# PKU-Alignment/Safe-Policy-Optimization

Hardware: NVIDIA H100
Metric: env-steps/sec PPO-Lag SafetyPointGoal1 @1024 envs/GPU (higher is better)
Workload: dtype f32

## Files before the change

safe-policy-optimization_b200/csrc/spo_update.cu:

```cuda
#include "spo_update_kernel.cuh"

#ifdef SPO_PHASE_TIMERS
extern "C" int spo_debug_phase_cycles(unsigned long long* out_16x24, int reset) {
  SPO_CUDA_TRY(cudaMemcpyFromSymbol(out_16x24, g_phase_cycles, sizeof(unsigned long long) * 16 * 24));
  if (reset) {
    unsigned long long z[16 * 24] = {0};
    SPO_CUDA_TRY(cudaMemcpyToSymbol(g_phase_cycles, z, sizeof(z)));
  }
  return SPO_OK;
}
#endif

extern "C" int spo_comm_slot_floats(const spo_dims* d, int* slot_floats) {
  int rc = spo_check_dims(d);
  if (rc) return rc;
  SPO_REQUIRE(slot_floats, SPO_ERR_INVALID_ARG, "spo_comm_slot_floats: null output");
  const int nt1 = d->obs_dim <= 64 ? 1 : 2;
  *slot_floats = NQ * dp_slot_words(nt1) * 2;
  return SPO_OK;
}

extern "C" int spo_pg_update(const spo_dims* d, float* params, float* adam_m, float* adam_v, int* adam_t,
                             const spo_batch* data, const int64_t* perm, int64_t perm_len, int batch,
                             spo_loss_kind kind, const spo_hparams* hp, spo_update_ctrl* ctrl, void* stream) {
// ... 31 lines not shown
    a.kind = SPO_LOSS_PPO_CLIP;
    a.hp.clip_lo = -INFINITY;
    a.hp.clip_hi = INFINITY;
  }
  if (comm && comm->world > 1) {
    SPO_REQUIRE(comm->rank >= 0 && comm->rank < comm->world && comm->world <= 16 && comm->grad_bufs,
                SPO_ERR_INVALID_ARG, "spo_pg_update_dp: bad spo_comm (world=%d rank=%d)", comm->world, comm->rank);
    SPO_REQUIRE(d->act_dim <= 8, SPO_ERR_UNSUPPORTED,
                "spo_pg_update_dp: act_dim=%d > 8 is single-GPU only (the cross-GPU update supports act_dim <= 8)", d->act_dim);
    a.comm = *comm;
  } else {
    a.comm.world = 1;
  }
  cudaStream_t st = static_cast<cudaStream_t>(stream);
  const bool dp = a.comm.world > 1;
  if (d->act_dim > 8) return spo_update_launch_wide(d->obs_dim <= 64 ? 1 : 2, &a, st);
  if (d->obs_dim <= 64) return dp ? launch_update<1, 8, true>(a, st) : launch_update<1, 8, false>(a, st);
  return dp ? launch_update<2, 8, true>(a, st) : launch_update<2, 8, false>(a, st);
}
```

safe-policy-optimization_b200/csrc/spo_update_kernel.cuh:

```cuda
#pragma once
#include <cooperative_groups.h>
#include <stdlib.h>
#include "spo_common.cuh"
#include "spo_mma.cuh"

namespace cg = cooperative_groups;

#ifdef SPO_PHASE_TIMERS
__device__ unsigned long long g_phase_cycles[16][24];
#define PHASE_MARK(idx)                                                   \
  do {                                                                    \
    if (tid == 0) {                                                       \
      const long long now__ = clock64();                                  \
      sm_phase__[idx] += static_cast<unsigned long long>(now__ - phase_t__); \
      phase_t__ = now__;                                                  \
    }                                                                     \
  } while (0)
#else
#define PHASE_MARK(idx) do { } while (0)
#endif

namespace {

constexpr int UT = 256;
constexpr int NQ = 4;
constexpr int SL = SPO_HID / NQ;
constexpr int NCTA = 3 * NQ;
constexpr int LDA = 72;
constexpr int LDS = 40;
constexpr float kLogSqrt2Pi = 0.91893853320467274178f;

template <int AC>
struct UpdShape {
  static_assert(AC == 8 || AC == 16, "action capacity 8 or 16");
  static constexpr int AUXW = 3 * AC + 4;
  static constexpr int AUX_LOGP = AC, AUX_ADV = AC + 1, AUX_TGT = AC + 2, AUX_OMEAN = AC + 4, AUX_OSTD = 2 * AC + 4;
  static constexpr int AUX_IT = (AUXW + 3) / 4;
  static constexpr int SP_B1 = 0, SP_B2 = SL, SP_W3 = 2 * SL, SP_B3 = 2 * SL + AC * SL, SP_LS = SP_B3 + AC;
  static constexpr int SPN = SP_LS + AC;
  static constexpr int SPT = (SPN + UT - 1) / UT;
  static constexpr int YQ = SPO_ROWS * AC;
  static constexpr int DH = AC / 4;
};
static_assert(UpdShape<8>::SPN == 176 && UpdShape<8>::SPT == 1 && UpdShape<16>::SPN == 320 && UpdShape<16>::SPT == 2, "layout");

__host__ __device__ constexpr int upd_ldx(int nt1) { return 64 * nt1 + 8; }
__host__ __device__ constexpr int dp_slot_words(int nt1) { return UT * 4 * (1 + nt1) + UT; }

template <int N> struct IC { static constexpr int value = N; };

struct UpdArgs {
  float *params, *adam_m, *adam_v;
  int* adam_t;
  spo_batch data;
  const int64_t* perm;
  int64_t perm_len;
  int batch, kind, D, A;
  int actor_only;
  spo_hparams hp;
  spo_update_ctrl* ctrl;
  spo_comm comm;
};

__device__ __forceinline__ uint32_t smem_u32(const void* p) { return static_cast<uint32_t>(__cvta_generic_to_shared(p)); }
__device__ __forceinline__ uint32_t mapa(uint32_t addr, uint32_t rank) {
  uint32_t r;
  asm volatile("mapa.shared::cluster.u32 %0, %1, %2;" : "=r"(r) : "r"(addr), "r"(rank));
  return r;
// ... 18 lines not shown
  while (!ok) {
    asm volatile("{ .reg .pred p; mbarrier.try_wait.parity.acquire.cluster.shared::cta.b64 p, [%1], %2; selp.u32 %0, 1, 0, p; }"
                 : "=r"(ok) : "r"(a), "r"(parity) : "memory");
  }
}
__device__ __forceinline__ void st_async16(uint32_t remote_dst, float4 v, uint32_t remote_bar) {
  asm volatile("st.async.shared::cluster.mbarrier::complete_tx::bytes.v4.b32 [%0], {%1, %2, %3, %4}, [%5];"
               ::"r"(remote_dst), "r"(__float_as_uint(v.x)), "r"(__float_as_uint(v.y)), "r"(__float_as_uint(v.z)),
               "r"(__float_as_uint(v.w)), "r"(remote_bar) : "memory");
}
__device__ __forceinline__ void bulk_push(uint32_t remote_dst, const void* local_src, uint32_t bytes, uint32_t remote_bar) {
  asm volatile("cp.async.bulk.shared::cluster.shared::cta.mbarrier::complete_tx::bytes [%0], [%1], %2, [%3];"
               ::"r"(remote_dst), "r"(smem_u32(local_src)), "r"(bytes), "r"(remote_bar) : "memory");
}
__device__ __forceinline__ void fence_proxy_async() { asm volatile("fence.proxy.async.shared::cta;" ::: "memory"); }
__device__ __forceinline__ void cp_async8(void* smem, const void* gmem) {
  asm volatile("cp.async.ca.shared.global [%0], [%1], 8;\n" ::"r"(smem_u32(smem)), "l"(gmem));
}
__device__ __forceinline__ void cp_async_commit() { asm volatile("cp.async.commit_group;\n" ::); }
__device__ __forceinline__ void cp_async_wait_all() { asm volatile("cp.async.wait_group 0;\n" ::: "memory"); }
__device__ __forceinline__ void st_ll(float2* p, float v, unsigned seq) {
  asm volatile("st.relaxed.sys.global.v2.b32 [%0], {%1, %2};" ::"l"(p), "r"(__float_as_uint(v)), "r"(seq) : "memory");
}

struct AdamK {
  float w1, b2, w2, ibc2s, eps, ss;
};
__device__ __forceinline__ float sqrt_approx(float x) {
  float r;
  asm("sqrt.approx.f32 %0, %1;" : "=f"(r) : "f"(x));
  return r;
}
__device__ __forceinline__ float adam_update(float p, float g, float& m, float& v, const AdamK& k) {
  m = fmaf(k.w1, __fsub_rn(g, m), m);
  v = __fadd_rn(__fmul_rn(v, k.b2), __fmul_rn(__fmul_rn(k.w2, g), g));
// ... 135 lines not shown
#pragma unroll
  for (int ks = 0; ks < 8; ++ks) {
    uint32_t ah[4], al[4], bh[2], bl[2];
#pragma unroll
    for (int i = 0; i < 4; ++i) spo_split_tf32(af[ks][i], ah[i], al[i]);
    spo_split_tf32(bf[ks][0], bh[0], bl[0]);
    spo_split_tf32(bf[ks][1], bh[1], bl[1]);
    spo_mma_tf32(c_lh, al, bh);
    spo_mma_tf32(c_hl, ah, bl);
    spo_mma_tf32(c_hh, ah, bh);
  }
#pragma unroll
  for (int e = 0; e < 4; ++e) acc[0][e] += (c_lh[e] + c_hl[e]) + c_hh[e];
}

template <int NT1, int AC, bool DP>
__global__ void __launch_bounds__(UT, 1) spo_update_kernel(const UpdArgs a) {
  static_assert(!(DP && AC != 8), "the cross-GPU gradient slots hold one small parameter per thread");
  using S = UpdShape<AC>;
  constexpr int AUXW = S::AUXW, AUX_LOGP = S::AUX_LOGP, AUX_ADV = S::AUX_ADV, AUX_TGT = S::AUX_TGT, AUX_OMEAN = S::AUX_OMEAN,
                AUX_OSTD = S::AUX_OSTD;
  constexpr int SP_B1 = S::SP_B1, SP_B2 = S::SP_B2, SP_W3 = S::SP_W3, SP_B3 = S::SP_B3, SP_LS = S::SP_LS, SPN = S::SPN;
  constexpr int SPT = S::SPT, YQ = S::YQ, DH = S::DH;
  extern __shared__ __align__(16) float smem[];
  __shared__ __align__(8) uint64_t bar_h1, bar_dh, bar_y, bar_ss[2];
  __shared__ int comm_dead;
  cg::cluster_group cluster = cg::this_cluster();
  const unsigned rank = cluster.block_rank();
  const int tid = threadIdx.x, lane = tid & 31, wid = tid >> 5;
  spo_update_ctrl* ctrl = a.ctrl;
  if (*reinterpret_cast<volatile int*>(&ctrl->stop)) return;

  const int D = a.D, A = a.A;
  constexpr int ldx = upd_ldx(NT1);
  const bool idle = rank >= NCTA;
  const int net = idle ? 2 : static_cast<int>(rank) / NQ;
  const int q = static_cast<int>(rank) % NQ;
  const unsigned grp0 = static_cast<unsigned>(net * NQ);
  const bool is_actor = (net == 0);
  const bool active = !idle && !(is_actor && a.kind == SPO_LOSS_CRITIC_ONLY) && !(!is_actor && a.actor_only);
  const SpoNetOff off = spo_net_off(D, A, net);
  const int O = off.out;
  const int g8 = lane >> 2, t4 = lane & 3;

  float* p = smem;
  int64_t* idxbuf = reinterpret_cast<int64_t*>(p); p += 2 * 2 * SPO_ROWS;
  float* lsc = p; p += 4 * AC;
  float* adk = p; p += 16;
  float* w1s = p; p += SL * ldx;
  float* w2s = p; p += SL * LDA;
  float* sp = p;  p += SPN;
  float* gsmall = p; p += SPN;
  float* x = p;   p += SPO_ROWS * ldx;
  float* aux = p; p += SPO_ROWS * AUXW;
  float* h1 = p;  p += NQ * H1Q;
  float* h2s = p; p += SPO_ROWS * LDS;
  float* dz2s = p; p += SPO_ROWS * LDS;
  float* dz1s = p; p += SPO_ROWS * LDS;
  float* yblk = p; p += NQ * YQ;
  float* y = p;   p += SPO_ROWS * AC;
  float* dy = p;  p += SPO_ROWS * AC;
  float* dls = p; p += SPO_ROWS * AC;
  float* dh1b = p; p += NQ * H1Q;
  float* dh1in = p; p += NQ * H1Q;
  float* red = p; p += 64;
  float* bk = p;  p += 3 * (4 * NT1 + 1) * UT;
  float* xin = p; p += 2 * 16 * 4;
  float* b1s = sp + SP_B1; float* b2s = sp + SP_B2; float* w3s = sp + SP_W3; float* b3 = sp + SP_B3; float* log_std = sp + SP_LS;

  const int tps = (a.batch + SPO_ROWS - 1) / SPO_ROWS;
  const int64_t n_steps = (a.perm_len + a.batch - 1) / a.batch;
  const int64_t n_tiles = n_steps * tps;

  if (tid == 0) {
    comm_dead = 0;
    mbar_init(&bar_h1, 1);
    mbar_init(&bar_dh, 1);
    mbar_init(&bar_y, 1);
    mbar_init(&bar_ss[0], 1);
    mbar_init(&bar_ss[1], 1);
    asm volatile("fence.mbarrier_init.release.cluster;" ::: "memory");
    if (!idle) { mbar_expect_tx(&bar_ss[0], (NCTA - 1) * 16); mbar_expect_tx(&bar_ss[1], (NCTA - 1) * 16); }
    for (int b = 0; b < 2; ++b) {
      adk[8 * b + 0] = static_cast<float>(1.0 - static_cast<double>(a.hp.beta1));
      adk[8 * b + 1] = a.hp.beta2;
      adk[8 * b + 2] = static_cast<float>(1.0 - static_cast<double>(a.hp.beta2));
      adk[8 * b + 4] = a.hp.adam_eps;
    }
    if (active) {
      mbar_expect_tx(&bar_h1, (NQ - 1) * H1Q * 4);
      mbar_expect_tx(&bar_dh, (NQ - 1) * H1Q * 4);
      mbar_expect_tx(&bar_y, (NQ - 1) * YQ * 4);
    }
  }

  bool sp_valid = false, sp_counted = false;
  int sp_goff = 0;
  if (tid < SPN && !idle) {
    const int i = tid;
    sp_counted = true;
    if (i < SP_B2) { sp_valid = true; sp_goff = off.b1 + SL * q + i; }
    else if (i < SP_W3) { sp_valid = true; sp_goff = off.b2 + SL * q + (i - SP_B2); }
    else if (i < SP_B3) { const int o = (i - SP_W3) / SL, kk = (i - SP_W3) % SL; sp_valid = o < O; sp_goff = off.w3 + o * SPO_HID + SL * q + kk; }
    else if (i < SP_LS) { const int o = i - SP_B3; sp_valid = o < O; sp_goff = off.b3 + o; sp_counted = (q == 0); }
    else { const int j = i - SP_LS; sp_valid = is_actor && j < A; sp_goff = off.log_std + j; sp_counted = (q == 0); }
  }
  float sp_m = 0.f, sp_v = 0.f;
// ... 20 lines not shown
      const int j = i / LDA, k = i - j * LDA;
      w2s[i] = (k < SPO_HID) ? __ldg(a.params + off.w2 + (SL * q + j) * SPO_HID + k) : 0.f;
    }
    if (tid < SPN) {
      sp[tid] = sp_valid ? a.params[sp_goff] : 0.f;
      gsmall[tid] = 0.f;
      if (sp_valid) { sp_m = a.adam_m[sp_goff]; sp_v = a.adam_v[sp_goff]; }
    }
    if constexpr (SPT > 1) {
      if (tid + UT < SPN) {
        sp[tid + UT] = sp_valid1 ? a.params[sp_goff1] : 0.f;
        gsmall[tid + UT] = 0.f;
        if (sp_valid1) { sp_m1 = a.adam_m[sp_goff1]; sp_v1 = a.adam_v[sp_goff1]; }
      }
    }
    for (int i = tid; i < SPO_ROWS * ldx; i += UT) x[i] = 0.f;
    for (int i = tid; i < SPO_ROWS * AUXW; i += UT) aux[i] = 0.f;
  }
  float mW2[4], vW2[4], mW1[NT1][4], vW1[NT1][4];
  auto frag_jk = [&](int e, int ntile, int& j, int& k) { j = g8 + ((e >> 1) << 3); k = 8 * ntile + 2 * t4 + (e & 1); };
#pragma unroll
  for (int e = 0; e < 4; ++e) {
    int j, k;
    frag_jk(e, wid, j, k);
    mW2[e] = active ? a.adam_m[off.w2 + (SL * q + j) * SPO_HID + k] : 0.f;
    vW2[e] = active ? a.adam_v[off.w2 + (SL * q + j) * SPO_HID + k] : 0.f;
#pragma unroll
    for (int i = 0; i < NT1; ++i) {
      frag_jk(e, wid + 8 * i, j, k);
      const bool ok = active && k < D;
      mW1[i][e] = ok ? a.adam_m[off.w1 + (SL * q + j) * D + k] : 0.f;
      vW1[i][e] = ok ? a.adam_v[off.w1 + (SL * q + j) * D + k] : 0.f;
    }
  }
  const int t0 = a.adam_t[net];
  double b1pow = pow(static_cast<double>(a.hp.beta1), static_cast<double>(t0));
  double b2pow = pow(static_cast<double>(a.hp.beta2), static_cast<double>(t0));
  const float lr = (net == 0) ? a.hp.lr_actor : (net == 1 ? a.hp.lr_reward : a.hp.lr_cost);
  const float extra_sumsq = (is_actor && q == 0 && a.kind == SPO_LOSS_CRITIC_ONLY && !idle) ? ctrl->extra_sumsq : 0.f;
  const float vcoef = (net == 1) ? a.hp.value_coef : 1.f;
  const float reg = is_actor ? 0.f : __fmul_rn(vcoef, __fmul_rn(a.hp.critic_l2, 2.f));

  constexpr int PF_MAX = 4 * NT1;
  const bool vec_rows = (D & 3) == 0;
  float xr[4 * PF_MAX];
#pragma unroll
  for (int i = 0; i < 4 * PF_MAX; ++i) xr[i] = 0.f;
  constexpr int AUX_IT = S::AUX_IT;
  float auxr[AUX_IT];
#pragma unroll
  for (int i = 0; i < AUX_IT; ++i) auxr[i] = 0.f;
  const int r4s = tid >> 2, q4s = tid & 3;
  const int aux_per = !is_actor ? 1 : A + 2 + (a.kind == SPO_LOSS_FOCOPS ? 2 * A : 0);
  auto aux_slot = [&](int c) {
    if (!is_actor) return AUX_TGT;
    if (c < A) return c;
    if (c == A) return AUX_LOGP;
    if (c == A + 1) return AUX_ADV;
    if (c < 2 * A + 2) return AUX_OMEAN + (c - A - 2);
    return AUX_OSTD + (c - 2 * A - 2);
  };
  auto aux_by_row = [&](int c) { return is_actor && (c < A || c >= A + 2); };
  auto aux_src = [&](int c) -> const float* {
    if (!is_actor) return (net == 1) ? a.data.target_r : a.data.target_c;
    if (c < A) return a.data.act + c;
    if (c == A) return a.data.logp;
    if (c == A + 1) return a.data.adv;
    if (c < 2 * A + 2) return a.data.old_mean + (c - A - 2);
    return a.data.old_std + (c - 2 * A - 2);
  };
  const float* aux_src0 = aux_src(q4s < aux_per ? q4s : 0);
  const int aux_mul0 = aux_by_row(q4s) ? A : 1;
  const int aux_slot0 = aux_slot(q4s < aux_per ? q4s : 0);

  int64_t step_idx = 0;
#ifdef SPO_PHASE_TIMERS
  __shared__ unsigned long long sm_phase__[24];
  if (tid < 24) sm_phase__[tid] = 0ull;
  long long phase_t__ = clock64();
#endif
  auto tile_after = [&](int64_t step, int sub, int n, int64_t& step_o, int& sub_o) {
    step_o = step; sub_o = sub;
    for (int i = 0; i < n; ++i)
      if (++sub_o == tps) { sub_o = 0; ++step_o; }
  };
  auto load_next = [&](int64_t qt, int64_t step, int sub) {
    if (!active || qt >= n_tiles) return;
    int64_t rs = a.perm_len - step * a.batch;
    if (rs > a.batch) rs = a.batch;
    int rows = static_cast<int>(rs) - sub * SPO_ROWS;
    rows = rows < 0 ? 0 : (rows > SPO_ROWS ? SPO_ROWS : rows);
    const uint32_t* ridx = reinterpret_cast<const uint32_t*>(idxbuf + (qt & 1) * SPO_ROWS);
    const uint32_t Du = static_cast<uint32_t>(D);
    const bool rv = r4s < rows;
    const uint32_t g = rv ? ridx[2 * r4s] : 0u;
    const float* rowp = a.data.obs + static_cast<size_t>(g) * Du;
    if (vec_rows) {
#pragma unroll
      for (int it = 0; it < PF_MAX; ++it) {
        const int c = q4s + 4 * it;
        float4 v = make_float4(0.f, 0.f, 0.f, 0.f);
        if (rv && 4 * c < D) v = __ldg(reinterpret_cast<const float4*>(rowp) + c);
        xr[4 * it] = v.x; xr[4 * it + 1] = v.y; xr[4 * it + 2] = v.z; xr[4 * it + 3] = v.w;
      }
    } else {
#pragma unroll
      for (int it = 0; it < 4 * PF_MAX; ++it) {
        const int c = q4s + 4 * it;
        xr[it] = (rv && c < D) ? __ldg(rowp + c) : 0.f;
      }
    }
    auxr[0] = (rv && q4s < aux_per) ? __ldg(aux_src0 + static_cast<size_t>(g) * static_cast<uint32_t>(aux_mul0)) : 0.f;
    if (aux_per > 4) {
#pragma unroll
      for (int i = 1; i < AUX_IT; ++i) {
        const int c = q4s + 4 * i;
        float v = 0.f;
        if (rv && c < aux_per) v = __ldg(aux_src(c) + static_cast<size_t>(g) * static_cast<uint32_t>(aux_by_row(c) ? A : 1));
        auxr[i] = v;
      }
    }
  };
  auto store_next = [&]() {
    if (!active) return;
    if (vec_rows) {
#pragma unroll
      for (int it = 0; it < PF_MAX; ++it) {
        const int c = q4s + 4 * it;
        if (4 * c < D) *reinterpret_cast<float4*>(x + r4s * ldx + 4 * c) = make_float4(xr[4 * it], xr[4 * it + 1], xr[4 * it + 2], xr[4 * it + 3]);
      }
    } else {
#pragma unroll
      for (int it = 0; it < 4 * PF_MAX; ++it) {
        const int c = q4s + 4 * it;
        if (c < D) x[r4s * ldx + c] = xr[it];
      }
    }
    if (q4s < aux_per) aux[r4s * AUXW + aux_slot0] = auxr[0];
    if (aux_per > 4) {
#pragma unroll
      for (int i = 1; i < AUX_IT; ++i) {
        const int c = q4s + 4 * i;
        if (c < aux_per) aux[r4s * AUXW + aux_slot(c)] = auxr[i];
      }
    }
  };
  auto fetch_idx = [&](int64_t qt, int64_t step, int sub) {
    if (!active || qt >= n_tiles) return;
    const int64_t first = step * a.batch + sub * SPO_ROWS;
    int64_t rs = a.perm_len - first;
    if (rs > a.batch - sub * SPO_ROWS) rs = a.batch - sub * SPO_ROWS;
    if (tid < SPO_ROWS && tid < rs) cp_async8(idxbuf + (qt & 1) * SPO_ROWS + tid, a.perm + first + tid);
  };
  auto colsum_into = [&](const float* buf, float* dst) {
    const int c = tid >> 4, rg = tid & 15;
    float s = 0.f;
#pragma unroll
    for (int i = 0; i < 4; ++i) s += buf[(rg + 16 * i) * LDS + c];
    s += __shfl_xor_sync(0xffffffffu, s, 1);
    s += __shfl_xor_sync(0xffffffffu, s, 2);
    s += __shfl_xor_sync(0xffffffffu, s, 4);
    s += __shfl_xor_sync(0xffffffffu, s, 8);
    if (rg == 0) dst[c] += s;
  };

  {
    int64_t st; int sb;
    fetch_idx(0, 0, 0);
    cp_async_commit();
    cp_async_wait_all();
    __syncthreads();
    load_next(0, 0, 0);
    tile_after(0, 0, 1, st, sb);
    fetch_idx(1, st, sb);
    cp_async_commit();
  }

  uint32_t ph_x = 0;
  uint32_t tcount = 0;

  float gW2[1][4], gW1[NT1][4];
#pragma unroll
  for (int e = 0; e < 4; ++e) {
    gW2[0][e] = 0.f;
#pragma unroll
    for (int i = 0; i < NT1; ++i) gW1[i][e] = 0.f;
  }
  double acc_loss = 0.0;
  float step_loss = 0.f, step_aux0 = 0.f, step_aux1 = 0.f;

  const int world = DP ? a.comm.world : 1, me = DP ? a.comm.rank : 0;
// ... 186 lines not shown
      frag_jk(e, wid, j, kc);
      *reinterpret_cast<float2*>(w2s + j * LDA + kc) = w2v[e >> 1];
    }
    if (own0) { sp[tid] = spv; gsmall[tid] = 0.f; }
    if constexpr (SPT > 1) {
      if (tid + UT < SPN) { sp[tid + UT] = spv1; gsmall[tid + UT] = 0.f; }
    }
#pragma unroll
    for (int e = 0; e < 4; ++e) gW2[0][e] = 0.f;
  };

  int64_t step = 0;
  int sub = 0;
  auto next_tile = [&]() { if (++sub == tps) { sub = 0; ++step; } };
  for (int64_t qt = 0; qt < n_tiles; ++qt, next_tile()) {
    int64_t rs64 = a.perm_len - step * a.batch;
    if (rs64 > a.batch) rs64 = a.batch;
    const int rows_step = static_cast<int>(rs64);
    int rows = rows_step - sub * SPO_ROWS;
    rows = rows < 0 ? 0 : (rows > SPO_ROWS ? SPO_ROWS : rows);
    const bool last_tile = (sub == tps - 1);
    const float inv_b = __fdiv_rn(1.f, static_cast<float>(rows_step));
    const unsigned seq = static_cast<unsigned>(a.comm.seq_base + static_cast<unsigned long long>(step_idx) + 1ull);
    const int par = static_cast<int>(step_idx & 1);
    auto stage_next = [&]() {
      int64_t st; int sb;
      tile_after(step, sub, 1, st, sb);
      load_next(qt + 1, st, sb);
      PHASE_MARK(18);
      tile_after(st, sb, 1, st, sb);
      fetch_idx(qt + 2, st, sb);
      cp_async_commit();
    };
    auto dp_push = [&](const float* vals, auto n_c, int w0) {
      constexpr int n = decltype(n_c)::value;
      const size_t base = ((static_cast<size_t>(seq & 1u) * world + me) * NCTA + rank) * DPW;
      for (int r = 0; r < world; ++r) {
        if (r == me) continue;
        float2* dst = reinterpret_cast<float2*>(a.comm.grad_bufs[r]) + base;
#pragma unroll
        for (int i = 0; i < n; ++i) st_ll(dst + (w0 + i) * UT + tid, vals[i], seq);
      }
    };
    auto dp_sum_wide = [&](float (&g2)[4], float (&g1)[NT1][4], float& gs) {
      constexpr int NW = 4 * (1 + NT1) + 1, G = 3;
      const unsigned limit = a.comm.spin_limit ? a.comm.spin_limit : 400000000u;
      const float inv_w = __fdiv_rn(1.f, static_cast<float>(world));
      float val[NW];
// ... 91 lines not shown
          }
        }
#pragma unroll
        for (int i = 0; i < NW; ++i) acc[i] += v[i];
      }
      const float inv_w = __fdiv_rn(1.f, static_cast<float>(world));
#pragma unroll
      for (int e = 0; e < 4; ++e) {
        g2[e] = __fmul_rn(acc[e], inv_w);
#pragma unroll
        for (int i = 0; i < NT1; ++i) g1[i][e] = __fmul_rn(acc[4 * (1 + i) + e], inv_w);
      }
      gs = __fmul_rn(acc[NW - 1], inv_w);
    };

    store_next();
    __syncthreads();
    PHASE_MARK(0);

    if (active) layer1();
    PHASE_MARK(2);
    const bool defer = pending;
    float clip = 1.f;
    if (pending) {
      pending = false;
      step_barrier_wait();
      PHASE_MARK(9);
      clip = resolve_clip(pend_par);
      if (active) {
        if (clip < 1.f) {
          __syncthreads();
// ... 57 lines not shown
#pragma unroll
      for (int h = 0; h < DH; ++h) piv[h] = 1.f;
#pragma unroll
      for (int h = 0; h < DH; ++h) pls[h] = 0.f;
      {
        const float* axp = aux + r4 * AUXW;
        if (is_actor) {
#pragma unroll
          for (int h = 0; h < DH; ++h) {
            const int j = k4 + 4 * h;
            if (j < A) { pa[h] = axp[j]; psd[h] = lsc[4 * j]; piv[h] = lsc[4 * j + 1]; pls[h] = lsc[4 * j + 2]; }
          }
          plogp = axp[AUX_LOGP];
          padv = axp[AUX_ADV];
        } else if (k4 == 0) {
          ptgt = axp[AUX_TGT];
        }
      }
      if (defer) log_loss(pend_par, pend_inv_b);
      if (last_tile) {
        float* kp = adk + 8 * par;
        if (tid == UT - 32) {
          b1pow *= static_cast<double>(a.hp.beta1);
          kp[5] = -__fdiv_rn(lr, static_cast<float>(1.0 - b1pow));
        } else if (tid == UT - 64) {
          b2pow *= static_cast<double>(a.hp.beta2);
          kp[3] = __fdiv_rn(1.f, sqrtf(static_cast<float>(1.0 - b2pow)));
        }
      }
      mbar_wait(&bar_y, ph_x);
      if (tid == 0) mbar_expect_tx(&bar_y, (NQ - 1) * YQ * 4);
// ... 261 lines not shown
          v[d] = *reinterpret_cast<const float4*>(src + r4 * SL + 4 * k4);
        }
        float4 s4 = v[0];
#pragma unroll
        for (int d = 1; d < NQ; ++d) { s4.x += v[d].x; s4.y += v[d].y; s4.z += v[d].z; s4.w += v[d].w; }
        const float4 h = *reinterpret_cast<const float4*>(h1 + q * H1Q + r4 * SL + ((4 * k4) ^ (((r4 >> 1) & 1) << 3)));
        s4.x *= (1.f - h.x * h.x); s4.y *= (1.f - h.y * h.y); s4.z *= (1.f - h.z * h.z); s4.w *= (1.f - h.w * h.w);
        *reinterpret_cast<float4*>(dz1s + r4 * LDS + 4 * k4) = s4;
      }
      __syncthreads();
      PHASE_MARK(11);
#pragma unroll
      for (int i = 0; i < NT1; ++i)
        warp_gemm<1, 8, true>(reinterpret_cast<float (&)[1][4]>(gW1[i]), dz1s, 1, LDS, x, ldx, 1, 0, (wid + 8 * i) * 8);
      colsum_into(dz1s, gsmall + SP_B1);
      PHASE_MARK(12);
    }

    cp_async_wait_all();
    __syncthreads();
    ph_x ^= active ? 1u : 0u;
    if (!last_tile) {
      step_barrier_push(par, 0.f, 0.f);
      stage_next();
      step_barrier_wait();
      continue;
    }

    if (DP && world > 1 && active) {
      float sv = 0.f;
      if (tid < SP_B2) { sv = gsmall[tid]; dp_push(&sv, IC<1>{}, 4 * (1 + NT1)); }
#pragma unroll
      for (int i = 0; i < NT1; ++i) dp_push(gW1[i], IC<4>{}, 4 * (1 + i));
      sv = (tid < SPN) ? gsmall[tid] : 0.f;
      stage_next();
      if (world >= 4 && world <= 8) dp_sum_wide(gW2[0], gW1, sv);
      else dp_sum_all(gW2[0], gW1, sv);
      if (tid < SPN) gsmall[tid] = sv;
    }
    PHASE_MARK(13);

    if (active) {
      float ss = 0.f, th2 = 0.f;
#pragma unroll
      for (int e = 0; e < 4; ++e) {
        int j, k;
        frag_jk(e, wid, j, k);
        if (!is_actor) {
          const float th = w2s[j * LDA + k];
          gW2[0][e] = fmaf(reg, th, gW2[0][e]);
// ... 35 lines not shown
      __syncthreads();
    }
    {
      float s = 0.f, t2 = 0.f;
      if (tid < NCTA && active) {
#pragma unroll
        for (int w = 0; w < UT / 32; w += 2) {
          const float4 v = *reinterpret_cast<const float4*>(red + 16 + 2 * w);
          s += v.x + v.z; t2 += v.y + v.w;
        }
      }
      PHASE_MARK(14);
      step_barrier_push(par, s + extra_sumsq, t2);
      PHASE_MARK(17);
    }
    if (!(DP && world > 1 && active)) stage_next();
    PHASE_MARK(15);
    if (active) adam_l1(1.f, true, adam_k(par));
    pending = true;
    pend_par = par;
    pend_inv_b = inv_b;
    PHASE_MARK(16);
    ++step_idx;
  }
  if (pending) {
    __syncthreads();
    step_barrier_wait();
    const float clip = resolve_clip(pend_par);
    if (active) {
      if (clip < 1.f) {
        __syncthreads();
        adam_l1_restore();
        adam_l1(clip, false, adam_k(pend_par));
      }
      log_loss(pend_par, pend_inv_b);
      adam_rest(clip, adam_k(pend_par));
    }
  }
  cp_async_wait_all();
  __syncthreads();

  if (active) {
    for (int i = tid; i < SL * D; i += UT) {
      const int j = i / D, kx = i - j * D;
      a.params[off.w1 + (SL * q + j) * D + kx] = w1s[j * ldx + kx];
    }
    for (int i = tid; i < SL * SPO_HID; i += UT)
      a.params[off.w2 + (SL * q + (i >> 6)) * SPO_HID + (i & 63)] = w2s[(i >> 6) * LDA + (i & 63)];
    if (tid < SPN && sp_valid && (sp_counted || tid < SP_B3)) {
      a.params[sp_goff] = sp[tid];
      a.adam_m[sp_goff] = sp_m;
      a.adam_v[sp_goff] = sp_v;
    }
    if constexpr (SPT > 1) {
// ... 19 lines not shown
      }
    }
    if (tid == 0 && q == 0) {
      a.adam_t[net] = t0 + static_cast<int>(n_steps);
      const int slot = (net == 0) ? 2 : (net == 1 ? 0 : 1);
      atomicAdd(&ctrl->loss_sum[slot], acc_loss);
    }
  }
#ifdef SPO_PHASE_TIMERS
  if (tid < 24) atomicAdd(&g_phase_cycles[rank & 15][tid], sm_phase__[tid]);
#endif
  if (rank == NQ && tid == 0) atomicAdd(reinterpret_cast<unsigned long long*>(&ctrl->steps), static_cast<unsigned long long>(n_steps));
  cluster.sync();
}

template <int AC>
size_t update_smem_bytes(int nt1) {
  using S = UpdShape<AC>;
  const int ldx = upd_ldx(nt1);
  size_t f = 4 * SPO_ROWS + 4 * AC + 16 + SL * ldx + SL * LDA + 2 * S::SPN + SPO_ROWS * ldx + SPO_ROWS * S::AUXW + NQ * SPO_ROWS * SL +
             3 * SPO_ROWS * LDS + (3 + NQ) * SPO_ROWS * AC + 2 * NQ * SPO_ROWS * SL + 64 + 128 + 3 * (4 * nt1 + 1) * UT;
  return f * sizeof(float);
}

template <int NT1, int AC, bool DP>
int launch_update(const UpdArgs& a, cudaStream_t stream) {
  const size_t smem = update_smem_bytes<AC>(NT1);
  SPO_REQUIRE(smem <= 227 * 1024, SPO_ERR_UNSUPPORTED, "spo_pg_update: obs_dim=%d needs %zu B of shared memory (> 227 KB)", a.D, smem);
  static int cluster_size = 0;
  SPO_CUDA_TRY(cudaFuncSetAttribute(spo_update_kernel<NT1, AC, DP>, cudaFuncAttributeMaxDynamicSharedMemorySize, static_cast<int>(smem)));
  SPO_CUDA_TRY(cudaFuncSetAttribute(spo_update_kernel<NT1, AC, DP>, cudaFuncAttributeNonPortableClusterSizeAllowed, 1));
  if (!cluster_size) {
    const char* env = getenv("SPO_CLUSTER");
    if (env && atoi(env) >= NCTA && atoi(env) <= 16) cluster_size = atoi(env);
  }
  for (int attempt = 0; attempt < 2; ++attempt) {
    const int cs = cluster_size ? cluster_size : (attempt == 0 ? NCTA : 16);
    cudaLaunchConfig_t cfg{};
    cfg.gridDim = dim3(cs);
    cfg.blockDim = dim3(UT);
    cfg.dynamicSmemBytes = smem;
    cfg.stream = stream;
    cudaLaunchAttribute attr[1];
// ... 2 lines not shown
    attr[0].val.clusterDim.y = 1;
    attr[0].val.clusterDim.z = 1;
    cfg.attrs = attr;
    cfg.numAttrs = 1;
    cudaError_t e = cudaLaunchKernelEx(&cfg, spo_update_kernel<NT1, AC, DP>, a);
    if (e == cudaSuccess) { cluster_size = cs; return SPO_OK; }
    if (cluster_size || attempt == 1) {
      spo_set_error("spo_pg_update: launch failed (cluster=%d): %s", cs, cudaGetErrorString(e));
      return SPO_ERR_CUDA;
    }
    (void)cudaGetLastError();
  }
  return SPO_ERR_CUDA;
}

}

int spo_update_launch_wide(int nt1, const void* args, cudaStream_t stream);
```

safe-policy-optimization_b200/csrc/spo_update_wide.cu:

```cuda
#undef SPO_PHASE_TIMERS
#include "spo_update_kernel.cuh"

int spo_update_launch_wide(int nt1, const void* args, cudaStream_t stream) {
  const UpdArgs& a = *static_cast<const UpdArgs*>(args);
  return nt1 == 1 ? launch_update<1, 16, false>(a, stream) : launch_update<2, 16, false>(a, stream);
}
```

Before: 216,600.

## Pre-pack minibatch tiles and stream them with TMA bulk copies

Adds a separate pack kernel that gathers permuted observation and auxiliary rows into contiguous padded tiles in a pooled global buffer. The update kernel then fetches each tile with a single cp.async.bulk into one of two shared-memory slots, tracked by mbarriers. This replaces the per-thread index fetch, register staging and store-to-smem pipeline. The cost is an extra kernel launch, a full copy of the batch through global memory, and a pool allocation per update. The aux layout also changes so critics read target_c from their own column.

```diff
diff --git a/safe-policy-optimization_b200/csrc/spo_update.cu b/safe-policy-optimization_b200/csrc/spo_update.cu
--- a/safe-policy-optimization_b200/csrc/spo_update.cu
+++ b/safe-policy-optimization_b200/csrc/spo_update.cu
@@ -1,4 +1,27 @@
+#include <mutex>
 #include "spo_update_kernel.cuh"
+
+int spo_update_tile_pool(cudaMemPool_t* pool) {
+  static std::mutex mu;
+  static cudaMemPool_t pools[64] = {};
+  int dev = 0;
+  SPO_CUDA_TRY(cudaGetDevice(&dev));
+  SPO_REQUIRE(dev >= 0 && dev < 64, SPO_ERR_UNSUPPORTED, "spo_pg_update: device %d", dev);
+  std::lock_guard<std::mutex> lock(mu);
+  if (!pools[dev]) {
+    cudaMemPoolProps props{};
+    props.allocType = cudaMemAllocationTypePinned;
+    props.location.type = cudaMemLocationTypeDevice;
+    props.location.id = dev;
+    cudaMemPool_t p;
+    SPO_CUDA_TRY(cudaMemPoolCreate(&p, &props));
+    uint64_t keep = UINT64_MAX;
+    SPO_CUDA_TRY(cudaMemPoolSetAttribute(p, cudaMemPoolAttrReleaseThreshold, &keep));
+    pools[dev] = p;
+  }
+  *pool = pools[dev];
+  return SPO_OK;
+}
 
 #ifdef SPO_PHASE_TIMERS
 extern "C" int spo_debug_phase_cycles(unsigned long long* out_16x24, int reset) {
@@ -69,7 +92,21 @@
   }
   cudaStream_t st = static_cast<cudaStream_t>(stream);
   const bool dp = a.comm.world > 1;
-  if (d->act_dim > 8) return spo_update_launch_wide(d->obs_dim <= 64 ? 1 : 2, &a, st);
+  if (d->act_dim > 8) return spo_update_launch_wide(d->obs_dim <= 64 ? 1 : 2, &a, st, false);
   if (d->obs_dim <= 64) return dp ? launch_update<1, 8, true>(a, st) : launch_update<1, 8, false>(a, st);
   return dp ? launch_update<2, 8, true>(a, st) : launch_update<2, 8, false>(a, st);
 }
+
+extern "C" int spo_debug_pack_tiles(const spo_dims* d, const spo_batch* data, const int64_t* perm, int64_t perm_len, int batch,
+                                    spo_loss_kind kind, spo_update_ctrl* ctrl, float* out, void* stream) {
+  int rc = spo_check_dims(d);
+  if (rc) return rc;
+  SPO_REQUIRE(data && perm && ctrl && out && batch > 0 && perm_len > 0, SPO_ERR_INVALID_ARG, "spo_debug_pack_tiles: bad argument");
+  UpdArgs a{};
+  a.tiles = out; a.data = *data; a.perm = perm; a.perm_len = perm_len; a.batch = batch; a.kind = kind;
+  a.D = d->obs_dim; a.A = d->act_dim; a.ctrl = ctrl;
+  cudaStream_t st = static_cast<cudaStream_t>(stream);
+  const int nt1 = d->obs_dim <= 64 ? 1 : 2;
+  if (d->act_dim > 8) return spo_update_launch_wide(nt1, &a, st, true);
+  return nt1 == 1 ? launch_pack<1, 8>(a, st) : launch_pack<2, 8>(a, st);
+}
diff --git a/safe-policy-optimization_b200/csrc/spo_update_kernel.cuh b/safe-policy-optimization_b200/csrc/spo_update_kernel.cuh
--- a/safe-policy-optimization_b200/csrc/spo_update_kernel.cuh
+++ b/safe-policy-optimization_b200/csrc/spo_update_kernel.cuh
@@ -5,6 +5,8 @@
 #include "spo_mma.cuh"
 
 namespace cg = cooperative_groups;
+
+int spo_update_tile_pool(cudaMemPool_t* pool);
 
 #ifdef SPO_PHASE_TIMERS
 __device__ unsigned long long g_phase_cycles[16][24];
@@ -35,7 +37,6 @@
   static_assert(AC == 8 || AC == 16, "action capacity 8 or 16");
   static constexpr int AUXW = 3 * AC + 4;
   static constexpr int AUX_LOGP = AC, AUX_ADV = AC + 1, AUX_TGT = AC + 2, AUX_OMEAN = AC + 4, AUX_OSTD = 2 * AC + 4;
-  static constexpr int AUX_IT = (AUXW + 3) / 4;
   static constexpr int SP_B1 = 0, SP_B2 = SL, SP_W3 = 2 * SL, SP_B3 = 2 * SL + AC * SL, SP_LS = SP_B3 + AC;
   static constexpr int SPN = SP_LS + AC;
   static constexpr int SPT = (SPN + UT - 1) / UT;
@@ -45,6 +46,10 @@
 static_assert(UpdShape<8>::SPN == 176 && UpdShape<8>::SPT == 1 && UpdShape<16>::SPN == 320 && UpdShape<16>::SPT == 2, "layout");
 
 __host__ __device__ constexpr int upd_ldx(int nt1) { return 64 * nt1 + 8; }
+template <int NT1, int AC>
+__host__ __device__ constexpr int upd_tile_floats() { return SPO_ROWS * (upd_ldx(NT1) + UpdShape<AC>::AUXW); }
+static_assert(upd_tile_floats<1, 8>() * 4 == 25600 && upd_tile_floats<2, 8>() * 4 == 41984 && upd_tile_floats<2, 16>() * 4 % 16 == 0,
+              "bulk copies move multiples of 16 bytes");
 __host__ __device__ constexpr int dp_slot_words(int nt1) { return UT * 4 * (1 + nt1) + UT; }
 
 template <int N> struct IC { static constexpr int value = N; };
@@ -52,6 +57,7 @@
 struct UpdArgs {
   float *params, *adam_m, *adam_v;
   int* adam_t;
+  float* tiles;
   spo_batch data;
   const int64_t* perm;
   int64_t perm_len;
@@ -100,11 +106,13 @@
                ::"r"(remote_dst), "r"(smem_u32(local_src)), "r"(bytes), "r"(remote_bar) : "memory");
 }
 __device__ __forceinline__ void fence_proxy_async() { asm volatile("fence.proxy.async.shared::cta;" ::: "memory"); }
-__device__ __forceinline__ void cp_async8(void* smem, const void* gmem) {
-  asm volatile("cp.async.ca.shared.global [%0], [%1], 8;\n" ::"r"(smem_u32(smem)), "l"(gmem));
-}
-__device__ __forceinline__ void cp_async_commit() { asm volatile("cp.async.commit_group;\n" ::); }
-__device__ __forceinline__ void cp_async_wait_all() { asm volatile("cp.async.wait_group 0;\n" ::: "memory"); }
+__device__ __forceinline__ void bulk_load(void* smem_dst, const void* gmem_src, uint32_t bytes, uint64_t* bar) {
+  asm volatile("cp.async.bulk.shared::cluster.global.mbarrier::complete_tx::bytes [%0], [%1], %2, [%3];"
+               ::"r"(smem_u32(smem_dst)), "l"(gmem_src), "r"(bytes), "r"(smem_u32(bar)) : "memory");
+}
+__device__ __forceinline__ void bulk_prefetch_l2(const void* gmem_src, uint32_t bytes) {
+  asm volatile("cp.async.bulk.prefetch.L2.global [%0], %1;" ::"l"(gmem_src), "r"(bytes) : "memory");
+}
 __device__ __forceinline__ void st_ll(float2* p, float v, unsigned seq) {
   asm volatile("st.relaxed.sys.global.v2.b32 [%0], {%1, %2};" ::"l"(p), "r"(__float_as_uint(v)), "r"(seq) : "memory");
 }
@@ -270,6 +278,58 @@
   for (int e = 0; e < 4; ++e) acc[0][e] += (c_lh[e] + c_hl[e]) + c_hh[e];
 }
 
+template <int NT1, int AC>
+__host__ __device__ constexpr size_t update_fixed_smem_bytes() {
+  using S = UpdShape<AC>;
+  return sizeof(float) * (4 * AC + 16 + SL * upd_ldx(NT1) + SL * LDA + 2 * S::SPN + NQ * SPO_ROWS * SL + 3 * SPO_ROWS * LDS +
+                          (3 + NQ) * SPO_ROWS * AC + 2 * NQ * SPO_ROWS * SL + 64 + 128 + 3 * (4 * NT1 + 1) * UT);
+}
+template <int NT1, int AC>
+__host__ __device__ constexpr int update_nslot() {
+  return update_fixed_smem_bytes<NT1, AC>() + 2 * sizeof(float) * upd_tile_floats<NT1, AC>() <= 227 * 1024 ? 2 : 1;
+}
+template <int NT1, int AC>
+__host__ __device__ constexpr size_t update_smem_bytes() {
+  return update_fixed_smem_bytes<NT1, AC>() + update_nslot<NT1, AC>() * sizeof(float) * upd_tile_floats<NT1, AC>();
+}
+static_assert(update_smem_bytes<1, 8>() == 172352 && update_smem_bytes<2, 8>() == 221504 && update_smem_bytes<1, 16>() == 200256 &&
+              update_smem_bytes<2, 16>() == 201280, "shared-memory figures in the comment above");
+
+template <int NT1, int AC>
+__global__ void __launch_bounds__(256) spo_pack_tiles(const UpdArgs a, int64_t n_tiles) {
+  using S = UpdShape<AC>;
+  if (*reinterpret_cast<volatile int*>(&a.ctrl->stop)) return;
+  constexpr int ldx = upd_ldx(NT1), AUXW = S::AUXW, TILEF = upd_tile_floats<NT1, AC>();
+  const int D = a.D, A = a.A, lane = threadIdx.x & 31;
+  const int tps = (a.batch + SPO_ROWS - 1) / SPO_ROWS;
+  const bool actor = a.kind != SPO_LOSS_CRITIC_ONLY, focops = a.kind == SPO_LOSS_FOCOPS;
+  const int64_t n_rows = n_tiles * SPO_ROWS, wstride = (static_cast<int64_t>(gridDim.x) * blockDim.x) >> 5;
+  for (int64_t w = (static_cast<int64_t>(blockIdx.x) * blockDim.x + threadIdx.x) >> 5; w < n_rows; w += wstride) {
+    const int64_t t = w / SPO_ROWS, step = t / tps;
+    const int r = static_cast<int>(w - t * SPO_ROWS), row = static_cast<int>(t - step * tps) * SPO_ROWS + r;
+    int64_t rows_step = a.perm_len - step * a.batch;
+    if (rows_step > a.batch) rows_step = a.batch;
+    const bool valid = row < rows_step;
+    const int64_t g = valid ? a.perm[step * a.batch + row] : 0;
+    float* xo = a.tiles + t * TILEF + r * ldx;
+    float* ao = a.tiles + t * TILEF + SPO_ROWS * ldx + r * AUXW;
+    const float* xs = a.data.obs + g * D;
+    for (int c = lane; c < ldx; c += 32) xo[c] = (valid && c < D) ? xs[c] : 0.f;
+    for (int c = lane; c < AUXW; c += 32) {
+      const float* src = nullptr;
+      int64_t i = g;
+      if (c < A) { if (actor) { src = a.data.act; i = g * A + c; } }
+      else if (c == S::AUX_LOGP) { if (actor) src = a.data.logp; }
+      else if (c == S::AUX_ADV) { if (actor) src = a.data.adv; }
+      else if (c == S::AUX_TGT) src = a.data.target_r;
+      else if (c == S::AUX_TGT + 1) src = a.data.target_c;
+      else if (c >= S::AUX_OMEAN && c < S::AUX_OMEAN + A) { if (focops) { src = a.data.old_mean; i = g * A + c - S::AUX_OMEAN; } }
+      else if (c >= S::AUX_OSTD && c < S::AUX_OSTD + A) { if (focops) { src = a.data.old_std; i = g * A + c - S::AUX_OSTD; } }
+      ao[c] = (valid && src) ? src[i] : 0.f;
+    }
+  }
+}
+
 template <int NT1, int AC, bool DP>
 __global__ void __launch_bounds__(UT, 1) spo_update_kernel(const UpdArgs a) {
   static_assert(!(DP && AC != 8), "the cross-GPU gradient slots hold one small parameter per thread");
@@ -278,8 +338,11 @@
                 AUX_OSTD = S::AUX_OSTD;
   constexpr int SP_B1 = S::SP_B1, SP_B2 = S::SP_B2, SP_W3 = S::SP_W3, SP_B3 = S::SP_B3, SP_LS = S::SP_LS, SPN = S::SPN;
   constexpr int SPT = S::SPT, YQ = S::YQ, DH = S::DH;
+  constexpr int NSLOT = update_nslot<NT1, AC>(), TILEF = upd_tile_floats<NT1, AC>();
+  constexpr uint32_t TILEB = TILEF * sizeof(float);
   extern __shared__ __align__(16) float smem[];
   __shared__ __align__(8) uint64_t bar_h1, bar_dh, bar_y, bar_ss[2];
+  __shared__ __align__(8) uint64_t bar_tile[NSLOT];
   __shared__ int comm_dead;
   cg::cluster_group cluster = cg::this_cluster();
   const unsigned rank = cluster.block_rank();
@@ -300,15 +363,15 @@
   const int g8 = lane >> 2, t4 = lane & 3;
 
   float* p = smem;
-  int64_t* idxbuf = reinterpret_cast<int64_t*>(p); p += 2 * 2 * SPO_ROWS;
   float* lsc = p; p += 4 * AC;
   float* adk = p; p += 16;
   float* w1s = p; p += SL * ldx;
   float* w2s = p; p += SL * LDA;
   float* sp = p;  p += SPN;
   float* gsmall = p; p += SPN;
-  float* x = p;   p += SPO_ROWS * ldx;
-  float* aux = p; p += SPO_ROWS * AUXW;
+  float* slots = p; p += NSLOT * TILEF;
+  float* x = slots;
+  float* aux = x + SPO_ROWS * ldx;
   float* h1 = p;  p += NQ * H1Q;
   float* h2s = p; p += SPO_ROWS * LDS;
   float* dz2s = p; p += SPO_ROWS * LDS;
@@ -327,6 +390,13 @@
   const int tps = (a.batch + SPO_ROWS - 1) / SPO_ROWS;
   const int64_t n_steps = (a.perm_len + a.batch - 1) / a.batch;
   const int64_t n_tiles = n_steps * tps;
+  auto issue_tile = [&](int64_t t) {
+    if (t >= n_tiles) return;
+    const int s = static_cast<int>(t % NSLOT);
+    mbar_expect_tx(&bar_tile[s], TILEB);
+    bulk_load(slots + s * TILEF, a.tiles + t * TILEF, TILEB, &bar_tile[s]);
+    if (NSLOT == 1 && t + 1 < n_tiles) bulk_prefetch_l2(a.tiles + (t + 1) * TILEF, TILEB);
+  };
 
   if (tid == 0) {
     comm_dead = 0;
@@ -335,6 +405,8 @@
     mbar_init(&bar_y, 1);
     mbar_init(&bar_ss[0], 1);
     mbar_init(&bar_ss[1], 1);
+#pragma unroll
+    for (int s = 0; s < NSLOT; ++s) mbar_init(&bar_tile[s], 1);
     asm volatile("fence.mbarrier_init.release.cluster;" ::: "memory");
     if (!idle) { mbar_expect_tx(&bar_ss[0], (NCTA - 1) * 16); mbar_expect_tx(&bar_ss[1], (NCTA - 1) * 16); }
     for (int b = 0; b < 2; ++b) {
@@ -347,6 +419,8 @@
       mbar_expect_tx(&bar_h1, (NQ - 1) * H1Q * 4);
       mbar_expect_tx(&bar_dh, (NQ - 1) * H1Q * 4);
       mbar_expect_tx(&bar_y, (NQ - 1) * YQ * 4);
+#pragma unroll
+      for (int t = 0; t < NSLOT; ++t) issue_tile(t);
     }
   }
 
@@ -397,8 +471,6 @@
         if (sp_valid1) { sp_m1 = a.adam_m[sp_goff1]; sp_v1 = a.adam_v[sp_goff1]; }
       }
     }
-    for (int i = tid; i < SPO_ROWS * ldx; i += UT) x[i] = 0.f;
-    for (int i = tid; i < SPO_ROWS * AUXW; i += UT) aux[i] = 0.f;
   }
   float mW2[4], vW2[4], mW1[NT1][4], vW1[NT1][4];
   auto frag_jk = [&](int e, int ntile, int& j, int& k) { j = g8 + ((e >> 1) << 3); k = 8 * ntile + 2 * t4 + (e & 1); };
@@ -424,117 +496,12 @@
   const float vcoef = (net == 1) ? a.hp.value_coef : 1.f;
   const float reg = is_actor ? 0.f : __fmul_rn(vcoef, __fmul_rn(a.hp.critic_l2, 2.f));
 
-  constexpr int PF_MAX = 4 * NT1;
-  const bool vec_rows = (D & 3) == 0;
-  float xr[4 * PF_MAX];
-#pragma unroll
-  for (int i = 0; i < 4 * PF_MAX; ++i) xr[i] = 0.f;
-  constexpr int AUX_IT = S::AUX_IT;
-  float auxr[AUX_IT];
-#pragma unroll
-  for (int i = 0; i < AUX_IT; ++i) auxr[i] = 0.f;
-  const int r4s = tid >> 2, q4s = tid & 3;
-  const int aux_per = !is_actor ? 1 : A + 2 + (a.kind == SPO_LOSS_FOCOPS ? 2 * A : 0);
-  auto aux_slot = [&](int c) {
-    if (!is_actor) return AUX_TGT;
-    if (c < A) return c;
-    if (c == A) return AUX_LOGP;
-    if (c == A + 1) return AUX_ADV;
-    if (c < 2 * A + 2) return AUX_OMEAN + (c - A - 2);
-    return AUX_OSTD + (c - 2 * A - 2);
-  };
-  auto aux_by_row = [&](int c) { return is_actor && (c < A || c >= A + 2); };
-  auto aux_src = [&](int c) -> const float* {
-    if (!is_actor) return (net == 1) ? a.data.target_r : a.data.target_c;
-    if (c < A) return a.data.act + c;
-    if (c == A) return a.data.logp;
-    if (c == A + 1) return a.data.adv;
-    if (c < 2 * A + 2) return a.data.old_mean + (c - A - 2);
-    return a.data.old_std + (c - 2 * A - 2);
-  };
-  const float* aux_src0 = aux_src(q4s < aux_per ? q4s : 0);
-  const int aux_mul0 = aux_by_row(q4s) ? A : 1;
-  const int aux_slot0 = aux_slot(q4s < aux_per ? q4s : 0);
-
   int64_t step_idx = 0;
 #ifdef SPO_PHASE_TIMERS
   __shared__ unsigned long long sm_phase__[24];
   if (tid < 24) sm_phase__[tid] = 0ull;
   long long phase_t__ = clock64();
 #endif
-  auto tile_after = [&](int64_t step, int sub, int n, int64_t& step_o, int& sub_o) {
-    step_o = step; sub_o = sub;
-    for (int i = 0; i < n; ++i)
-      if (++sub_o == tps) { sub_o = 0; ++step_o; }
-  };
-  auto load_next = [&](int64_t qt, int64_t step, int sub) {
-    if (!active || qt >= n_tiles) return;
-    int64_t rs = a.perm_len - step * a.batch;
-    if (rs > a.batch) rs = a.batch;
-    int rows = static_cast<int>(rs) - sub * SPO_ROWS;
-    rows = rows < 0 ? 0 : (rows > SPO_ROWS ? SPO_ROWS : rows);
-    const uint32_t* ridx = reinterpret_cast<const uint32_t*>(idxbuf + (qt & 1) * SPO_ROWS);
-    const uint32_t Du = static_cast<uint32_t>(D);
-    const bool rv = r4s < rows;
-    const uint32_t g = rv ? ridx[2 * r4s] : 0u;
-    const float* rowp = a.data.obs + static_cast<size_t>(g) * Du;
-    if (vec_rows) {
-#pragma unroll
-      for (int it = 0; it < PF_MAX; ++it) {
-        const int c = q4s + 4 * it;
-        float4 v = make_float4(0.f, 0.f, 0.f, 0.f);
-        if (rv && 4 * c < D) v = __ldg(reinterpret_cast<const float4*>(rowp) + c);
-        xr[4 * it] = v.x; xr[4 * it + 1] = v.y; xr[4 * it + 2] = v.z; xr[4 * it + 3] = v.w;
-      }
-    } else {
-#pragma unroll
-      for (int it = 0; it < 4 * PF_MAX; ++it) {
-        const int c = q4s + 4 * it;
-        xr[it] = (rv && c < D) ? __ldg(rowp + c) : 0.f;
-      }
-    }
-    auxr[0] = (rv && q4s < aux_per) ? __ldg(aux_src0 + static_cast<size_t>(g) * static_cast<uint32_t>(aux_mul0)) : 0.f;
-    if (aux_per > 4) {
-#pragma unroll
-      for (int i = 1; i < AUX_IT; ++i) {
-        const int c = q4s + 4 * i;
-        float v = 0.f;
-        if (rv && c < aux_per) v = __ldg(aux_src(c) + static_cast<size_t>(g) * static_cast<uint32_t>(aux_by_row(c) ? A : 1));
-        auxr[i] = v;
-      }
-    }
-  };
-  auto store_next = [&]() {
-    if (!active) return;
-    if (vec_rows) {
-#pragma unroll
-      for (int it = 0; it < PF_MAX; ++it) {
-        const int c = q4s + 4 * it;
-        if (4 * c < D) *reinterpret_cast<float4*>(x + r4s * ldx + 4 * c) = make_float4(xr[4 * it], xr[4 * it + 1], xr[4 * it + 2], xr[4 * it + 3]);
-      }
-    } else {
-#pragma unroll
-      for (int it = 0; it < 4 * PF_MAX; ++it) {
-        const int c = q4s + 4 * it;
-        if (c < D) x[r4s * ldx + c] = xr[it];
-      }
-    }
-    if (q4s < aux_per) aux[r4s * AUXW + aux_slot0] = auxr[0];
-    if (aux_per > 4) {
-#pragma unroll
-      for (int i = 1; i < AUX_IT; ++i) {
-        const int c = q4s + 4 * i;
-        if (c < aux_per) aux[r4s * AUXW + aux_slot(c)] = auxr[i];
-      }
-    }
-  };
-  auto fetch_idx = [&](int64_t qt, int64_t step, int sub) {
-    if (!active || qt >= n_tiles) return;
-    const int64_t first = step * a.batch + sub * SPO_ROWS;
-    int64_t rs = a.perm_len - first;
-    if (rs > a.batch - sub * SPO_ROWS) rs = a.batch - sub * SPO_ROWS;
-    if (tid < SPO_ROWS && tid < rs) cp_async8(idxbuf + (qt & 1) * SPO_ROWS + tid, a.perm + first + tid);
-  };
   auto colsum_into = [&](const float* buf, float* dst) {
     const int c = tid >> 4, rg = tid & 15;
     float s = 0.f;
@@ -546,18 +513,6 @@
     s += __shfl_xor_sync(0xffffffffu, s, 8);
     if (rg == 0) dst[c] += s;
   };
-
-  {
-    int64_t st; int sb;
-    fetch_idx(0, 0, 0);
-    cp_async_commit();
-    cp_async_wait_all();
-    __syncthreads();
-    load_next(0, 0, 0);
-    tile_after(0, 0, 1, st, sb);
-    fetch_idx(1, st, sb);
-    cp_async_commit();
-  }
 
   uint32_t ph_x = 0;
   uint32_t tcount = 0;
@@ -774,6 +729,8 @@
   int sub = 0;
   auto next_tile = [&]() { if (++sub == tps) { sub = 0; ++step; } };
   for (int64_t qt = 0; qt < n_tiles; ++qt, next_tile()) {
+    x = slots + (qt % NSLOT) * TILEF;
+    aux = x + SPO_ROWS * ldx;
     int64_t rs64 = a.perm_len - step * a.batch;
     if (rs64 > a.batch) rs64 = a.batch;
     const int rows_step = static_cast<int>(rs64);
@@ -783,15 +740,6 @@
     const float inv_b = __fdiv_rn(1.f, static_cast<float>(rows_step));
     const unsigned seq = static_cast<unsigned>(a.comm.seq_base + static_cast<unsigned long long>(step_idx) + 1ull);
     const int par = static_cast<int>(step_idx & 1);
-    auto stage_next = [&]() {
-      int64_t st; int sb;
-      tile_after(step, sub, 1, st, sb);
-      load_next(qt + 1, st, sb);
-      PHASE_MARK(18);
-      tile_after(st, sb, 1, st, sb);
-      fetch_idx(qt + 2, st, sb);
-      cp_async_commit();
-    };
     auto dp_push = [&](const float* vals, auto n_c, int w0) {
       constexpr int n = decltype(n_c)::value;
       const size_t base = ((static_cast<size_t>(seq & 1u) * world + me) * NCTA + rank) * DPW;
@@ -913,7 +861,7 @@
       gs = __fmul_rn(acc[NW - 1], inv_w);
     };
 
-    store_next();
+    if (active) mbar_wait(&bar_tile[qt % NSLOT], static_cast<uint32_t>(qt / NSLOT) & 1u);
     __syncthreads();
     PHASE_MARK(0);
 
@@ -1001,7 +949,7 @@
           plogp = axp[AUX_LOGP];
           padv = axp[AUX_ADV];
         } else if (k4 == 0) {
-          ptgt = axp[AUX_TGT];
+          ptgt = axp[AUX_TGT + (net == 2 ? 1 : 0)];
         }
       }
       if (defer) log_loss(pend_par, pend_inv_b);
@@ -1293,15 +1241,15 @@
       for (int i = 0; i < NT1; ++i)
         warp_gemm<1, 8, true>(reinterpret_cast<float (&)[1][4]>(gW1[i]), dz1s, 1, LDS, x, ldx, 1, 0, (wid + 8 * i) * 8);
       colsum_into(dz1s, gsmall + SP_B1);
+      fence_proxy_async();
       PHASE_MARK(12);
     }
 
-    cp_async_wait_all();
     __syncthreads();
+    if (active && tid == UT - 32) issue_tile(qt + NSLOT);
     ph_x ^= active ? 1u : 0u;
     if (!last_tile) {
       step_barrier_push(par, 0.f, 0.f);
-      stage_next();
       step_barrier_wait();
       continue;
     }
@@ -1312,7 +1260,6 @@
 #pragma unroll
       for (int i = 0; i < NT1; ++i) dp_push(gW1[i], IC<4>{}, 4 * (1 + i));
       sv = (tid < SPN) ? gsmall[tid] : 0.f;
-      stage_next();
       if (world >= 4 && world <= 8) dp_sum_wide(gW2[0], gW1, sv);
       else dp_sum_all(gW2[0], gW1, sv);
       if (tid < SPN) gsmall[tid] = sv;
@@ -1378,8 +1325,6 @@
       step_barrier_push(par, s + extra_sumsq, t2);
       PHASE_MARK(17);
     }
-    if (!(DP && world > 1 && active)) stage_next();
-    PHASE_MARK(15);
     if (active) adam_l1(1.f, true, adam_k(par));
     pending = true;
     pend_par = par;
@@ -1401,7 +1346,6 @@
       adam_rest(clip, adam_k(pend_par));
     }
   }
-  cp_async_wait_all();
   __syncthreads();
 
   if (active) {
@@ -1451,19 +1395,23 @@
   cluster.sync();
 }
 
-template <int AC>
-size_t update_smem_bytes(int nt1) {
-  using S = UpdShape<AC>;
-  const int ldx = upd_ldx(nt1);
-  size_t f = 4 * SPO_ROWS + 4 * AC + 16 + SL * ldx + SL * LDA + 2 * S::SPN + SPO_ROWS * ldx + SPO_ROWS * S::AUXW + NQ * SPO_ROWS * SL +
-             3 * SPO_ROWS * LDS + (3 + NQ) * SPO_ROWS * AC + 2 * NQ * SPO_ROWS * SL + 64 + 128 + 3 * (4 * nt1 + 1) * UT;
-  return f * sizeof(float);
+inline int64_t upd_n_tiles(const UpdArgs& a) {
+  return (a.perm_len + a.batch - 1) / a.batch * ((a.batch + SPO_ROWS - 1) / SPO_ROWS);
+}
+
+template <int NT1, int AC>
+int launch_pack(const UpdArgs& a, cudaStream_t stream) {
+  const int64_t n_tiles = upd_n_tiles(a);
+  const int64_t blocks = (n_tiles * SPO_ROWS + 7) / 8;
+  spo_pack_tiles<NT1, AC><<<static_cast<unsigned>(blocks < 65536 ? blocks : 65536), 256, 0, stream>>>(a, n_tiles);
+  SPO_CUDA_TRY(cudaGetLastError());
+  return SPO_OK;
 }
 
 template <int NT1, int AC, bool DP>
-int launch_update(const UpdArgs& a, cudaStream_t stream) {
-  const size_t smem = update_smem_bytes<AC>(NT1);
-  SPO_REQUIRE(smem <= 227 * 1024, SPO_ERR_UNSUPPORTED, "spo_pg_update: obs_dim=%d needs %zu B of shared memory (> 227 KB)", a.D, smem);
+int launch_update_kernel(const UpdArgs& a, cudaStream_t stream) {
+  constexpr size_t smem = update_smem_bytes<NT1, AC>();
+  static_assert(smem <= 227 * 1024, "shared memory of the update kernel");
   static int cluster_size = 0;
   SPO_CUDA_TRY(cudaFuncSetAttribute(spo_update_kernel<NT1, AC, DP>, cudaFuncAttributeMaxDynamicSharedMemorySize, static_cast<int>(smem)));
   SPO_CUDA_TRY(cudaFuncSetAttribute(spo_update_kernel<NT1, AC, DP>, cudaFuncAttributeNonPortableClusterSizeAllowed, 1));
@@ -1496,6 +1444,23 @@
   return SPO_ERR_CUDA;
 }
 
-}
-
-int spo_update_launch_wide(int nt1, const void* args, cudaStream_t stream);
+template <int NT1, int AC, bool DP>
+int launch_update(UpdArgs a, cudaStream_t stream) {
+  cudaMemPool_t pool;
+  int rc = spo_update_tile_pool(&pool);
+  if (rc) return rc;
+  const size_t bytes = static_cast<size_t>(upd_n_tiles(a)) * upd_tile_floats<NT1, AC>() * sizeof(float);
+  SPO_CUDA_TRY(cudaMallocFromPoolAsync(reinterpret_cast<void**>(&a.tiles), bytes, pool, stream));
+  rc = launch_pack<NT1, AC>(a, stream);
+  if (rc == SPO_OK) rc = launch_update_kernel<NT1, AC, DP>(a, stream);
+  const cudaError_t e = cudaFreeAsync(a.tiles, stream);
+  if (rc == SPO_OK && e != cudaSuccess) {
+    spo_set_error("spo_pg_update: cudaFreeAsync failed: %s", cudaGetErrorString(e));
+    return SPO_ERR_CUDA;
+  }
+  return rc;
+}
+
+}
+
+int spo_update_launch_wide(int nt1, const void* args, cudaStream_t stream, bool pack_only);
diff --git a/safe-policy-optimization_b200/csrc/spo_update_wide.cu b/safe-policy-optimization_b200/csrc/spo_update_wide.cu
--- a/safe-policy-optimization_b200/csrc/spo_update_wide.cu
+++ b/safe-policy-optimization_b200/csrc/spo_update_wide.cu
@@ -1,7 +1,8 @@
 #undef SPO_PHASE_TIMERS
 #include "spo_update_kernel.cuh"
 
-int spo_update_launch_wide(int nt1, const void* args, cudaStream_t stream) {
+int spo_update_launch_wide(int nt1, const void* args, cudaStream_t stream, bool pack_only) {
   const UpdArgs& a = *static_cast<const UpdArgs*>(args);
+  if (pack_only) return nt1 == 1 ? launch_pack<1, 16>(a, stream) : launch_pack<2, 16>(a, stream);
   return nt1 == 1 ? launch_update<1, 16, false>(a, stream) : launch_update<2, 16, false>(a, stream);
 }
```

After: 233,100, median of 6. 7.6% higher.
